# zhen6618/EPRecon

Measured on AMD Instinct MI355X. Metric: fragments_per_sec, higher is better.
Workload: dtype f32

## Files before the change

### eprecon_amd/_lib.py

```python
import ctypes
import os

import torch

_HERE = os.path.dirname(os.path.abspath(__file__))
LIB_PATH = os.environ.get("EPRECON_LIB_PATH") or os.path.join(_HERE, "libeprecon_hip.so")

_c = ctypes
_vp, _i, _i64, _f, _sz = _c.c_void_p, _c.c_int, _c.c_int64, _c.c_float, _c.c_size_t

SIGNATURES = {
    "eprecon_abi_version": (_i, []),
    "eprecon_build_arch": (_c.c_char_p, []),
    "eprecon_back_project_workspace_bytes": (_sz, [_i64, _i, _i, _i, _i, _i, _i]),
    "eprecon_back_project_async": (_i, [_vp, _i64, _vp, _i, _f, _vp, _i, _vp, _i, _i, _i, _i, _i, _i,
                                        _vp, _vp, _vp, _vp, _vp, _vp, _vp, _vp, _sz, _vp]),
    "eprecon_back_project": (_i, [_vp, _i64, _vp, _i, _f, _vp, _i, _vp, _i, _i, _i, _i, _i, _i, _i,
                                  _vp, _vp, _vp, _vp, _vp, _vp, _vp, _vp, _vp, _sz, _vp]),
    "eprecon_profile_gather_kernel": (_c.c_char_p, []),
    "eprecon_hash_capacity": (_c.c_uint32, [_i64]),
    "eprecon_hash_table_bytes": (_sz, [_c.c_uint32]),
    "eprecon_hash_build_async": (_i, [_vp, _i64, _i, _vp, _c.c_uint32, _vp]),
    "eprecon_hash_build_dn_async": (_i, [_vp, _i64, _vp, _i, _vp, _c.c_uint32, _vp]),
    "eprecon_hash_query_async": (_i, [_vp, _c.c_uint32, _vp, _i64, _i, _vp, _vp]),
    "eprecon_hash_status": (_i, [_vp, _vp]),
    "eprecon_unique_workspace_bytes": (_sz, [_i64]),
    "eprecon_unique_coords_async": (_i, [_vp, _i64, _i, _vp, _c.c_uint32, _vp, _vp, _vp, _vp, _sz, _vp]),
    "eprecon_unique_coords_dn_async": (_i, [_vp, _i64, _vp, _i, _vp, _c.c_uint32, _vp, _vp, _vp, _vp, _sz, _vp]),
    "eprecon_unique_hierarchy_dn_async": (_i, [_vp, _i64, _vp, _i, _vp, _vp, _vp, _vp, _vp, _vp, _sz, _vp]),
    "eprecon_point_quantize_dn_async": (_i, [_vp, _i64, _vp, _f, _vp, _vp, _vp]),
    "eprecon_spvcnn_points_dn_async": (_i, [_vp, _i64, _vp, _i, _i, _vp, _i, _f, _vp, _f, _vp, _vp, _vp, _vp, _vp, _vp]),
    "eprecon_gru_stage_capacity": (_i64, [_vp, _i64, _i]),
    "eprecon_gru_stage_workspace_bytes": (_sz, [_i64]),
    "eprecon_gru_stage_begin_async": (_i, [_vp, _vp]),
    "eprecon_gru_stage_commit_async": (_i, [_vp, _vp, _vp, _vp]),
    "eprecon_kernel_map_async": (_i, [_vp, _c.c_uint32, _vp, _i64, _i, _i, _vp, _vp]),
    "eprecon_kernel_map_self_async": (_i, [_vp, _c.c_uint32, _vp, _i64, _i, _vp, _vp]),
    "eprecon_transpose_map_async": (_i, [_vp, _i64, _vp, _i, _vp, _vp]),
    "eprecon_sparse_conv_async": (_i, [_vp, _i64, _i, _vp, _i, _i64, _vp, _i, _i, _vp, _vp, _i, _i, _i, _vp]),
    "eprecon_conv_bn_partial_bytes": (_sz, [_i64, _i]),
    "eprecon_sparse_conv_fused_async": (_i, [_vp, _i64, _i, _vp, _i, _i64, _vp, _i, _i, _vp, _vp, _i, _vp, _i, _i, _i,
                                             _vp, _vp]),
    "eprecon_conv_desc_async": (_i, [_vp, _vp]),
    "eprecon_exclusive_scan_async": (_i, [_vp, _i64, _vp, _vp, _vp, _vp]),
    "eprecon_conv_desc_partial_rows": (_i64, [_vp]),
    "eprecon_bn_acc_words": (_sz, [_i]),
    "eprecon_conv_desc_takes_bn_acc": (_i, [_vp]),
    "eprecon_batchnorm_acc_affine_async": (_i, [_vp, _i, _i, _i, _f, _vp, _vp, _vp]),
    "eprecon_affine_rows_acc_async": (_i, [_vp, _i64, _i, _i, _vp, _i, _i, _f, _i, _vp, _i, _vp]),
# ... 402 lines not shown
```

### eprecon_amd/back_project.py

```python
import ctypes

import torch
import torch.nn as nn

from . import _lib

MODE_MEAN, MODE_MEAN_DEPTH, MODE_VARIANCE = 0, 1, 2
LAYOUT_NCHW, LAYOUT_NHWC = 0, 1
def mark_dense(coords, dims, interval, batch=1):
    coords._eprecon_dense = (tuple(int(d) for d in dims), int(interval), int(batch))
    return coords


def _prep_feats(feats):
    v, b, c, h, w = feats.shape
    if feats.dtype != torch.float32:
        feats = feats.float()
    want = (b * h * w * c, h * w * c, 1, w * c, c)
    if all(sz == 1 or st == ws for sz, st, ws in zip(feats.shape, feats.stride(), want)):
        return feats, LAYOUT_NHWC
    return feats.contiguous(), LAYOUT_NCHW


class PendingBackProject:
# ... 150 lines not shown
    res = run(coords, origin, voxel_size, feats, KRcam, min_view_number, MODE_MEAN, min_valid_per_batch=0)
    if res is None:
        return torch.empty((0, feats.shape[2]), dtype=feats.dtype, device=feats.device)
    return res["feats"]


def forward_behind(module, coords, origin, voxel_size, feats, KRcam, min_view_number, behind):
    pend = run_async(coords, origin, voxel_size, feats, KRcam, min_view_number, MODE_MEAN, want_grid=module.return_projection,
                     hold_read=True, extra_words=behind.n_extra)
    nb = pend.n_valid_dev.numel() - behind.n_extra
    finish = behind(pend.coords_all, pend.n_valid_dev[0:1], pend.n_valid_dev[nb:])
    host = _lib.read_counts(pend.n_valid_dev)
    res = pend.result_from(host[:nb])
    if res is None:
        return None, None
    out_coords = res["coords"] if coords.dtype == torch.int32 else res["coords"].to(coords.dtype)
    return [res["feats"], out_coords, res.get("grid"), res.get("mask"), res["count"]], finish(res["n_valid"], host[nb:])


def view_variance(coords, origin, voxel_size, feats_fused, KRcam, min_view_number, min_valid=1000):
    if torch.is_grad_enabled() and feats_fused.requires_grad:
        from . import autograd as AG
        res = AG.back_project(coords, origin, voxel_size, feats_fused, KRcam, min_view_number, MODE_VARIANCE,
                              min_valid_per_batch=min_valid, want_mean=True)
    else:
        res = run(coords, origin, voxel_size, feats_fused, KRcam, min_view_number, MODE_VARIANCE,
                  min_valid_per_batch=min_valid, want_mean=True)
    if res is None:
        return None
    res["var"] = res.pop("feats")
    return res


def to_channels_last(feats):
    lib = _lib.load()
    v, b, c, h, w = feats.shape
    src = feats.float().contiguous()
    dst = torch.empty((v, b, h, w, c), dtype=torch.float32, device=feats.device)
    _lib.check(lib.eprecon_nchw_to_nhwc_async(_lib.ptr(src), _lib.ptr(dst), v * b, c, h * w,
                                               _lib.current_stream()), "eprecon_nchw_to_nhwc_async")
    return dst.permute(0, 1, 4, 2, 3)
```

### eprecon_amd/csrc/back_project.hip

```cpp
#include <stdlib.h>

#include "common.hpp"

namespace {
using namespace ep;


struct BpParams {
    const int32_t *coords;
    int n;
    const float *origin;
    int batch;
    float voxel_size;
    const float *feats_nhwc;
    const float *krcam;
    int V, C, H, W;
    int Cs;
    int min_view;
    float *out_feats;
    float *out_mean;
    int32_t *out_coords;
    float *count;
    float *out_grid;
    uint8_t *out_mask;
    int32_t *n_valid_dev;
    int32_t *block_offsets;
    int xcd_slabs;
};

struct Proj {
    float gx, gy, pz;
    bool vis;
};

__device__ __forceinline__ Proj project(const float *P, float X, float Y, float Z, float wm1,
                                        float hm1)
{
    const float px = __fmaf_rn(P[3], 1.0f, __fmaf_rn(P[2], Z, __fmaf_rn(P[1], Y, __fmul_rn(P[0], X))));
    const float py = __fmaf_rn(P[7], 1.0f, __fmaf_rn(P[6], Z, __fmaf_rn(P[5], Y, __fmul_rn(P[4], X))));
    const float pz = __fmaf_rn(P[11], 1.0f, __fmaf_rn(P[10], Z, __fmaf_rn(P[9], Y, __fmul_rn(P[8], X))));
    const float u = __fdiv_rn(px, pz);
    const float v = __fdiv_rn(py, pz);
    Proj r;
    r.gx = __fsub_rn(__fdiv_rn(__fmul_rn(2.0f, u), wm1), 1.0f);
    r.gy = __fsub_rn(__fdiv_rn(__fmul_rn(2.0f, v), hm1), 1.0f);
    r.pz = pz;
    r.vis = (fabsf(r.gx) <= 1.0f) && (fabsf(r.gy) <= 1.0f) && (pz > 0.0f);
    return r;
}

struct ProjFast {
    float u, v, pz;
    bool vis;
};

__device__ __forceinline__ ProjFast project_fast(const float *P, float X, float Y, float Z, float wm1, float hm1,
                                                 float kx, float ky)
{
    const float px = __fmaf_rn(P[3], 1.0f, __fmaf_rn(P[2], Z, __fmaf_rn(P[1], Y, __fmul_rn(P[0], X))));
// ... 117 lines not shown
        }
        if (lane == kWave - 1) sWave[wid] = x;
        __syncthreads();
        int woff = 0, tot = 0;
#pragma unroll
        for (int w = 0; w < 1024 / kWave; ++w) {
            const int c = sWave[w];
            woff += (w < wid) ? c : 0;
            tot += c;
        }
        if (i < nblk) block_sums[i] = carry + woff + x - v;
        carry += tot;
        __syncthreads();
    }
    if (tid == 0) n_valid_dev[0] = carry;
    if (batch == 1) {
        if (tid == 0) n_valid_dev[1] = carry;
    } else if (blk_batch) {
        for (int b = 0; b < batch; ++b) {
            int x = 0;
            for (int i = tid; i < nblk_count; i += 1024) x += blk_batch[(size_t)i * batch + b];
#pragma unroll
            for (int d = kWave / 2; d > 0; d >>= 1) x += __shfl_xor(x, d);
            __syncthreads();
            if (lane == 0) sWave[wid] = x;
            __syncthreads();
            if (tid == 0) {
                int t = 0;
                for (int w = 0; w < 1024 / kWave; ++w) t += sWave[w];
                n_valid_dev[1 + b] = t;
            }
        }
    }
}

struct Taps {
    int o00, o10, o01, o11;
    float w00, w10, w01, w11;
};

__device__ __forceinline__ Taps make_taps(float ix, float iy, int W, int H, int C)
{
    const float x0f = floorf(ix), y0f = floorf(iy);
    int x0 = (int)x0f, y0 = (int)y0f;
    float wx1 = ix - x0f, wx0 = (x0f + 1.0f) - ix;
    float wy1 = iy - y0f, wy0 = (y0f + 1.0f) - iy;
    int x1 = x0 + 1, y1 = y0 + 1;
    if (x1 >= W) { x1 = W - 1; wx1 = 0.0f; }
    if (y1 >= H) { y1 = H - 1; wy1 = 0.0f; }
    Taps t;
    t.o00 = (y0 * W + x0) * C;
    t.o10 = (y0 * W + x1) * C;
    t.o01 = (y1 * W + x0) * C;
    t.o11 = (y1 * W + x1) * C;
    t.w00 = wx0 * wy0;
    t.w10 = wx1 * wy0;
    t.w01 = wx0 * wy1;
    t.w11 = wx1 * wy1;
    return t;
}

template <int VEC>
struct Chan;
template <>
struct Chan<4> {
    float4 v;
// ... 32 lines not shown
};
template <>
struct Chan<1> {
    float v;
    __device__ __forceinline__ static Chan zero() { return Chan{0.f}; }
    __device__ __forceinline__ static Chan sample(const float *m, const Taps &t)
    {
        return Chan{fmaf(m[t.o11], t.w11, fmaf(m[t.o01], t.w01, fmaf(m[t.o10], t.w10, m[t.o00] * t.w00)))};
    }
    __device__ __forceinline__ void add(const Chan &o) { v += o.v; }
    __device__ __forceinline__ void add_sqdiff(const Chan &f, const Chan &mean)
    {
        const float d = f.v - mean.v;
        v = fmaf(d, d, v);
    }
    __device__ __forceinline__ Chan div(float d) const { return Chan{__fdiv_rn(v, d)}; }
    __device__ __forceinline__ void store(float *dst, bool) const { dst[0] = v; }
};

template <int VOX, int MODE, int VEC, int QT>
__global__ __launch_bounds__(256) void bp_gather_kernel(BpParams p)
{
    extern __shared__ __attribute__((aligned(16))) char smem[];
    constexpr int BLOCK = 256;
    float2 *sPix = reinterpret_cast<float2 *>(smem);
    float *sP = reinterpret_cast<float *>(sPix + VOX * p.V);
    const int nP = (p.V * p.batch * 12 + 3) & ~3;
    uint32_t *sVis = reinterpret_cast<uint32_t *>(sP + nP);
    float *sDen = reinterpret_cast<float *>(sVis + VOX);
    int *sBatch = reinterpret_cast<int *>(sDen + VOX);
    int *sSlot = sBatch + VOX;
    int *sOut = sSlot + VOX;
    int *sWave = sOut + VOX;

    const int tid = threadIdx.x;
    const int lb = p.xcd_slabs ? xcd_remap(blockIdx.x, gridDim.x) : (int)blockIdx.x;
    stage_matrices(sP, p.krcam, p.V * p.batch, tid, BLOCK);
    __syncthreads();

    const int e = lb * VOX + tid;
    const int i = e;
    const float wm1 = (float)(p.W - 1), hm1 = (float)(p.H - 1);
    bool valid = false;
    int4 c = make_int4(0, 0, 0, 0);
    float X = 0.f, Y = 0.f, Z = 0.f, zsum = 0.f;
    int cnt = 0;
    uint32_t vis = 0;
    if (tid < VOX && e < p.n) {
        c = reinterpret_cast<const int4 *>(p.coords)[i];
        if (c.x >= 0 && c.x < p.batch) {
            voxel_centre(c, p.origin, p.voxel_size, X, Y, Z);
            for (int v = 0; v < p.V; ++v) {
                const Proj pr = project(sP + (v * p.batch + c.x) * 12, X, Y, Z, wm1, hm1);
                const float ix = __fmul_rn(__fdiv_rn(__fadd_rn(pr.gx, 1.0f), 2.0f), wm1);
                const float iy = __fmul_rn(__fdiv_rn(__fadd_rn(pr.gy, 1.0f), 2.0f), hm1);
                sPix[tid * p.V + v] = make_float2(ix, iy);
                if (pr.vis) {
                    vis |= 1u << v;
                    cnt += 1;
                    zsum += pr.pz;
                }
            }
            valid = cnt >= p.min_view;
        }
    }
    int nloc;
    const int rank = block_exclusive_rank<BLOCK>(valid, sWave, nloc);
    if (nloc == 0) return;
    const int base = p.block_offsets[lb];
    const int n_valid = p.n_valid_dev[0];
    const int cout = (MODE == EPRECON_BP_MEAN_DEPTH) ? p.C + 1 : p.C;
    if (valid) {
        const int o = base + rank;
        sSlot[rank] = tid;
        sOut[tid] = o;
        sVis[tid] = vis;
        const float den = (float)(cnt > 0 ? cnt : 1);
        sDen[tid] = den;
        sBatch[tid] = c.x;
        reinterpret_cast<int4 *>(p.out_coords)[o] = c;
        if (MODE == EPRECON_BP_MEAN_DEPTH) p.out_feats[(size_t)o * cout + p.C] = __fdiv_rn(zsum, den);
        if (p.out_grid || p.out_mask) {
            for (int v = 0; v < p.V; ++v) {
                const Proj pr = project(sP + (v * p.batch + c.x) * 12, X, Y, Z, wm1, hm1);
                if (p.out_grid)
                    reinterpret_cast<float2 *>(p.out_grid)[(size_t)v * n_valid + o] = make_float2(pr.gx, pr.gy);
                if (p.out_mask) p.out_mask[(size_t)v * n_valid + o] = pr.vis ? 1 : 0;
            }
        }
    }
    __syncthreads();

    const int Q = QT > 0 ? QT : p.C / VEC;
    const size_t map_elems = (size_t)p.H * p.W * p.Cs;
    const bool aligned16 = (MODE != EPRECON_BP_MEAN_DEPTH);
    for (int w = tid; w < nloc * Q; w += BLOCK) {
        const int r = w / Q;
        const int q = w - r * Q;
        const int t = sSlot[r];
        const uint32_t vm = sVis[t];
        const float den = sDen[t];
        const int b = sBatch[t];
        const float *fb = p.feats_nhwc + (size_t)b * map_elems + q * VEC;
// ... 55 lines not shown
            a[u] = __builtin_amdgcn_raw_buffer_load_b128(rsrc, off[u], 0, 0);
            b[u] = __builtin_amdgcn_raw_buffer_load_b128(rsrc, off[u], s10, 0);
            c[u] = __builtin_amdgcn_raw_buffer_load_b128(rsrc, off[u], s01, 0);
            d[u] = __builtin_amdgcn_raw_buffer_load_b128(rsrc, off[u], s11, 0);
        }
#pragma unroll
        for (int u = 0; u < U; ++u) {
            const float wx1 = wxy[u].x, wy1 = wxy[u].y;
            const float wx0 = 1.0f - wx1, wy0 = 1.0f - wy1;
            const float w00 = wx0 * wy0, w10 = wx1 * wy0, w01 = wx0 * wy1, w11 = wx1 * wy1;
            float4 r;
#define EP_TAP(k) fmaf(__uint_as_float(d[u].k), w11, fmaf(__uint_as_float(c[u].k), w01, fmaf(__uint_as_float(b[u].k), w10, __uint_as_float(a[u].k) * w00)))
            r.x = EP_TAP(x); r.y = EP_TAP(y); r.z = EP_TAP(z); r.w = EP_TAP(w);
#undef EP_TAP
            if (on[u]) f(r);
        }
    }
}

template <int VOX, int MODE, int QT, int U>
__global__ __launch_bounds__(256) void bp_gather_mlp_kernel(BpParams p)
{
    extern __shared__ __attribute__((aligned(16))) char smem[];
    constexpr int BLOCK = 256;
    constexpr int VPT = BLOCK / VOX;
    float2 *sWxy = reinterpret_cast<float2 *>(smem);
    int *sOff = reinterpret_cast<int *>(sWxy + VOX * p.V);
    float *sP = reinterpret_cast<float *>(sOff + VOX * p.V);
    const int nP = (p.V * p.batch * 12 + 3) & ~3;
    uint32_t *sVis = reinterpret_cast<uint32_t *>(sP + nP);
    int *sSlot = reinterpret_cast<int *>(sVis + VOX);
    int *sOut = sSlot + VOX;
    int *sWave = sOut + VOX;

    const int tid = threadIdx.x;
    const int lb = p.xcd_slabs ? xcd_remap(blockIdx.x, gridDim.x) : (int)blockIdx.x;
    stage_matrices(sP, p.krcam, p.V * p.batch, tid, BLOCK);
    if (VPT > 1 && tid < VOX) sVis[tid] = 0;
    __syncthreads();

    const float wm1 = (float)(p.W - 1), hm1 = (float)(p.H - 1);
    const float kx = 2.0f / wm1, ky = 2.0f / hm1;
    const int map_elems = p.H * p.W * p.Cs;
    const int vx = tid % VOX;
    const int e = lb * VOX + vx;
    int4 c = make_int4(-1, 0, 0, 0);
    if (e < p.n) c = reinterpret_cast<const int4 *>(p.coords)[e];
    const bool in_batch = c.x >= 0 && c.x < p.batch;
    uint32_t vis = 0;
    if (in_batch) {
        float X, Y, Z;
        voxel_centre(c, p.origin, p.voxel_size, X, Y, Z);
        for (int v = tid / VOX; v < p.V; v += VPT) {
            const ProjFast q = project_fast(sP + (v * p.batch + c.x) * 12, X, Y, Z, wm1, hm1, kx, ky);
            if (!q.vis) continue;
            const float x0f = fminf(floorf(q.u), wm1 - 1.0f), y0f = fminf(floorf(q.v), hm1 - 1.0f);
            sWxy[vx * p.V + v] = make_float2(q.u - x0f, q.v - y0f);
            sOff[vx * p.V + v] = ((v * p.batch + c.x) * map_elems + ((int)y0f * p.W + (int)x0f) * p.Cs) * 4;
            vis |= 1u << v;
        }
        if (VPT > 1 && vis) atomicOr(&sVis[vx], vis);
    }
    if (VPT > 1) {
        __syncthreads();
        vis = sVis[vx];
    }
    const int cnt = __popc(vis);
    const bool valid = tid < VOX && in_batch && cnt >= p.min_view;
    int nloc;
    const int rank = block_exclusive_rank<BLOCK>(valid, sWave, nloc);
    if (nloc == 0) return;
    const int n_valid = p.n_valid_dev[0];
    const int cout = (MODE == EPRECON_BP_MEAN_DEPTH) ? p.C + 1 : p.C;
    if (valid) {
        const int o = p.block_offsets[lb] + rank;
        sSlot[rank] = tid;
        sOut[tid] = o;
        if (VPT == 1) sVis[tid] = vis;
        reinterpret_cast<int4 *>(p.out_coords)[o] = c;
        if (MODE == EPRECON_BP_MEAN_DEPTH || p.out_grid || p.out_mask) {
            float X, Y, Z, zsum = 0.0f;
            voxel_centre(c, p.origin, p.voxel_size, X, Y, Z);
            for (int v = 0; v < p.V; ++v) {
                const Proj pr = project(sP + (v * p.batch + c.x) * 12, X, Y, Z, wm1, hm1);
                if (pr.vis) zsum += pr.pz;
                if (p.out_grid)
                    reinterpret_cast<float2 *>(p.out_grid)[(size_t)v * n_valid + o] = make_float2(pr.gx, pr.gy);
                if (p.out_mask) p.out_mask[(size_t)v * n_valid + o] = pr.vis ? 1 : 0;
            }
            if (MODE == EPRECON_BP_MEAN_DEPTH)
                p.out_feats[(size_t)o * cout + p.C] = __fdiv_rn(zsum, (float)(cnt > 0 ? cnt : 1));
        }
    }
    __syncthreads();
    const __amdgpu_buffer_rsrc_t rsrc = __builtin_amdgcn_make_buffer_rsrc(
        const_cast<float *>(p.feats_nhwc), 0, p.V * p.batch * map_elems * 4, 0x00020000);
    const int Q = QT > 0 ? QT : p.C / 4;
    const int s10 = p.Cs * 4, s01 = p.W * p.Cs * 4, s11 = s01 + s10;
    for (int w = tid; w < nloc * Q; w += BLOCK) {
        const int r = w / Q, q = w - r * Q;
        const int t = sSlot[r];
        const uint32_t vm = sVis[t];
        const float den = (float)max(__popc(vm), 1);
        const int *offRow = sOff + t * p.V;
        const float2 *wxyRow = sWxy + t * p.V;
        float4 acc = make_float4(0.f, 0.f, 0.f, 0.f);
        visit_visible_samples<U>(rsrc, offRow, wxyRow, vm, q * 16, s10, s01, s11, [&](const float4 &f) {
            acc.x += f.x; acc.y += f.y; acc.z += f.z; acc.w += f.w;
// ... 34 lines not shown
    auto block_sum = [&](float x) -> float {
#pragma unroll
        for (int s = kWave / 2; s > 0; s >>= 1) x += __shfl_xor(x, s);
        __syncthreads();
        if (lane == 0) sRed[wid] = x;
        __syncthreads();
        float t = 0.f;
#pragma unroll
        for (int w = 0; w < 1024 / kWave; ++w) t += sRed[w];
        return t;
    };
    float s = 0.f, m = 0.f;
    for (int j = tid; j < len; j += 1024) {
        const float x = d[(size_t)j * cout];
        if (x > 0.f) { s += x; m += 1.f; }
    }
    const float tot = block_sum(s), cntp = block_sum(m);
    const float mu = tot / cntp;
    float ss = 0.f;
    for (int j = tid; j < len; j += 1024) {
        const float x = d[(size_t)j * cout];
        if (x > 0.f) ss = fmaf(x - mu, x - mu, ss);
    }
    const float sigma = sqrtf(block_sum(ss)) + 1e-5f;
    for (int j = tid; j < len; j += 1024) {
        const float x = d[(size_t)j * cout];
        d[(size_t)j * cout] = x > 0.f ? (x - mu) / sigma : 0.f;
    }
    (void)sBcast;
}

constexpr int kTrPix = 64;
__global__ __launch_bounds__(256) void nchw_to_nhwc_kernel(const float *__restrict__ in,
                                                           float *__restrict__ out, int C, int hw, int Cs,
                                                           int32_t *zero = nullptr, int zero_n = 0)
{
    extern __shared__ __attribute__((aligned(16))) char smem[];
    float *tile = reinterpret_cast<float *>(smem);
    if (blockIdx.x == 0 && blockIdx.y == 0 && (int)threadIdx.x < zero_n) zero[threadIdx.x] = 0;
    const int map = blockIdx.y;
    const int p0 = blockIdx.x * kTrPix;
    const int npix = min(kTrPix, hw - p0);
    const float *src = in + (size_t)map * C * hw;
    float *dst = out + (size_t)map * hw * Cs + (size_t)p0 * Cs;
    for (int e = threadIdx.x; e < C * kTrPix; e += 256) {
        const int c = e / kTrPix, px = e - c * kTrPix;
        if (px < npix) tile[c * (kTrPix + 1) + px] = src[(size_t)c * hw + p0 + px];
    }
    __syncthreads();
    for (int e = threadIdx.x; e < npix * Cs; e += 256) {
        const int px = e / Cs, c = e - px * Cs;
        dst[e] = c < C ? tile[c * (kTrPix + 1) + px] : 0.0f;
    }
}


struct ViewsParams {
    eprecon_views_desc d;
    int tile0[4];
    int tiles[3];
};
__global__ __launch_bounds__(256) void views_to_rows_kernel(ViewsParams p)
{
    extern __shared__ __attribute__((aligned(16))) char smem[];
    float *tile = reinterpret_cast<float *>(smem);
    const int b = blockIdx.x;
    const int l = b >= p.tile0[2] ? 2 : (b >= p.tile0[1] ? 1 : 0);
    const int r = b - p.tile0[l];
    const int v = r / p.tiles[l], t = r - v * p.tiles[l];
    const int C = p.d.channels[l], hw = p.d.hw[l];
    const int p0 = t * kTrPix;
    const int npix = min(kTrPix, hw - p0);
// ... 78 lines not shown
        const float iy = __fmul_rn(__fdiv_rn(__fadd_rn(pr.gy, 1.0f), 2.0f), hm1);
        const Taps t = make_taps(ix, iy, p.W, p.H, p.C);
        const size_t mo = ((size_t)v * p.batch + c.x) * map_elems + ch;
        float gv;
        if (p.mode == EPRECON_BP_VARIANCE) {
            const float f = Chan<1>::sample(p.feats_nhwc + mo, t).v;
            gv = 2.0f * (f - mean) * inv * g + gm;
        } else {
            gv = g * inv;
        }
        if (p.dfix) {
            unsigned long long *d = p.dfix + mo;
            float *m = p.dfeats + mo;
            if (t.w00 != 0.0f) fixed_add(d + t.o00, m + t.o00, t.w00 * gv);
            if (t.w10 != 0.0f) fixed_add(d + t.o10, m + t.o10, t.w10 * gv);
            if (t.w01 != 0.0f) fixed_add(d + t.o01, m + t.o01, t.w01 * gv);
            if (t.w11 != 0.0f) fixed_add(d + t.o11, m + t.o11, t.w11 * gv);
        } else {
            float *d = p.dfeats + mo;
            if (t.w00 != 0.0f) unsafeAtomicAdd(d + t.o00, t.w00 * gv);
            if (t.w10 != 0.0f) unsafeAtomicAdd(d + t.o10, t.w10 * gv);
            if (t.w01 != 0.0f) unsafeAtomicAdd(d + t.o01, t.w01 * gv);
            if (t.w11 != 0.0f) unsafeAtomicAdd(d + t.o11, t.w11 * gv);
        }
    }
}

struct ProfileState {
    bool on = false, recorded = false, one_shot = false;
    hipEvent_t start = nullptr, stop = nullptr;
    const char *kernel = "";
} g_prof;

size_t gather_lds_bytes(int vox, int V, int B)
{
    const size_t nP = ((size_t)V * B * 12 + 3) & ~(size_t)3;
    return (size_t)vox * V * sizeof(float2) + nP * sizeof(float) + (size_t)vox * 5 * 4 +
           (size_t)(256 / kWave) * 4 + 16;
}

template <int VOX, int MODE>
int launch_gather(const BpParams &p, int nblk, hipStream_t st)
{
    const size_t lds = gather_lds_bytes(VOX, p.V, p.batch);
    const dim3 grid(nblk), block(256);
#define EP_GATHER(VEC, QT) hipLaunchKernelGGL((bp_gather_kernel<VOX, MODE, VEC, QT>), grid, block, lds, st, p)
    if (p.C % 4 == 0) {
        switch (p.C / 4) {
            case 6: EP_GATHER(4, 6); break;
            case 8: EP_GATHER(4, 8); break;
            case 10: EP_GATHER(4, 10); break;
            case 20: EP_GATHER(4, 20); break;
            default: EP_GATHER(4, 0); break;
        }
    } else {
        EP_GATHER(1, 0);
    }
#undef EP_GATHER
    EP_LAUNCH_CHECK();
    return EPRECON_OK;
}

size_t gather_mlp_lds_bytes(int vox, int V, int B)
{
    const size_t nP = ((size_t)V * B * 12 + 3) & ~(size_t)3;
    return (size_t)vox * V * 12 + nP * sizeof(float) + (size_t)vox * 3 * 4 + (size_t)(256 / kWave) * 4 + 16;
}

bool gather_mlp_supported(const BpParams &p)
{
    return p.C % 4 == 0 && p.Cs % 4 == 0 && p.V <= 32 &&
           (size_t)p.V * p.batch * p.H * p.W * p.Cs * 4 < 0x7fff0000ull &&
           gather_mlp_lds_bytes(256, p.V, p.batch) <= 64 * 1024;
}

template <int VOX, int MODE, int U>
int launch_gather_mlp_u(const BpParams &p, int nblk, hipStream_t st)
{
    const size_t lds = gather_mlp_lds_bytes(VOX, p.V, p.batch);
    const dim3 grid(nblk), block(256);
#define EP_GATHER(QT) hipLaunchKernelGGL((bp_gather_mlp_kernel<VOX, MODE, QT, U>), grid, block, lds, st, p)
    switch (p.C / 4) {
        case 6: EP_GATHER(6); break;
        case 8: EP_GATHER(8); break;
        case 10: EP_GATHER(10); break;
        case 20: EP_GATHER(20); break;
        default: EP_GATHER(0); break;
    }
#undef EP_GATHER
    EP_LAUNCH_CHECK();
    return EPRECON_OK;
}

template <int VOX, int MODE>
int launch_gather_mlp(const BpParams &p, int nblk, hipStream_t st)
{
    return launch_gather_mlp_u<VOX, MODE, 1>(p, nblk, st);
}

// ... 63 lines not shown
    if (lds > 64 * 1024) return EPRECON_ERR_UNSUPPORTED;
    const dim3 grid((unsigned)ep::ceil_div(hw, kTrPix), (unsigned)maps);
    hipLaunchKernelGGL(nchw_to_nhwc_kernel, grid, dim3(256), lds, (hipStream_t)stream, in, out,
                       channels, hw, channels);
    EP_LAUNCH_CHECK();
    return EPRECON_OK;
}

int eprecon_views_to_rows_async(const eprecon_views_desc *desc, void *stream)
{
    if (!desc || desc->levels < 1 || desc->levels > 3 || desc->n_views < 1 || desc->n_views > 16) return EPRECON_ERR_ARG;
    ViewsParams p = {};
    p.d = *desc;
    int cmax = 0, at = 0;
    for (int l = 0; l < 3; ++l) {
        p.tile0[l] = at;
        if (l >= desc->levels) { p.tiles[l] = 1; continue; }
        if (desc->channels[l] <= 0 || desc->hw[l] <= 0 || !desc->dst[l]) return EPRECON_ERR_ARG;
        for (int v = 0; v < desc->n_views; ++v)
            if (!desc->src[l][v]) return EPRECON_ERR_ARG;
        p.tiles[l] = ep::ceil_div(desc->hw[l], kTrPix);
        at += p.tiles[l] * desc->n_views;
        cmax = desc->channels[l] > cmax ? desc->channels[l] : cmax;
    }
    p.tile0[3] = at;
    for (int l = desc->levels; l < 3; ++l) p.tile0[l] = at;
    const size_t lds = (size_t)cmax * (kTrPix + 1) * sizeof(float);
    if (lds > 64 * 1024) return EPRECON_ERR_UNSUPPORTED;
    hipLaunchKernelGGL(views_to_rows_kernel, dim3((unsigned)at), dim3(256), lds, (hipStream_t)stream, p);
    EP_LAUNCH_CHECK();
    return EPRECON_OK;
}

int eprecon_back_project_async(const int32_t *coords, int64_t n, const float *origin, int batch,
                               float voxel_size, const float *feats, int feats_layout,
                               const float *krcam, int n_views, int channels, int height,
                               int width, int min_view, int mode, float *out_feats,
                               float *out_mean, int32_t *out_coords, float *count,
                               float *out_grid, uint8_t *out_mask, int32_t *n_valid_dev,
                               void *workspace, size_t workspace_bytes, void *stream)
{
    hipStream_t st = (hipStream_t)stream;
    if (n < 0 || n > 0x7fffffff / 64 || batch <= 0 || n_views <= 0 || n_views > 32 || channels <= 0 ||
        height <= 1 || width <= 1 || mode < 0 || mode > 2)
        return EPRECON_ERR_ARG;
    if (!origin || !feats || !krcam || !n_valid_dev || !workspace) return EPRECON_ERR_ARG;
    if (n > 0 && (!coords || !out_feats || !out_coords || !count)) return EPRECON_ERR_ARG;
    if ((size_t)n_views * batch * 12 * sizeof(float) > 32 * 1024) return EPRECON_ERR_UNSUPPORTED;
    if (workspace_bytes < eprecon_back_project_workspace_bytes(n, batch, n_views, channels, height,
                                                               width, feats_layout))
        return EPRECON_ERR_WORKSPACE;
    if ((size_t)n_views * batch * channels * height * width > 0x7fffffffull) return EPRECON_ERR_UNSUPPORTED;

    const bool clear_in_relayout = n > 0 && feats_layout == EPRECON_LAYOUT_NCHW && batch < 256;
    if (!clear_in_relayout) EP_HIP_CHECK(hipMemsetAsync(n_valid_dev, 0, sizeof(int32_t) * (size_t)(1 + batch), st));
    if (n == 0) return EPRECON_OK;

    char *ws = reinterpret_cast<char *>(workspace);
    int32_t *block_sums = reinterpret_cast<int32_t *>(ws);
    ws += ep::align_up((size_t)ep::ceil_div(n, 16) * sizeof(int32_t), 256);
    int32_t *blk_batch = reinterpret_cast<int32_t *>(ws);
    ws += ep::align_up((size_t)ep::ceil_div(n, 256) * batch * sizeof(int32_t), 256);
    const float *nhwc = feats;
    int pix_stride = channels;
    if (feats_layout == EPRECON_LAYOUT_NCHW) {
        float *tmp = reinterpret_cast<float *>(ws);
        const size_t lds_t = (size_t)channels * (kTrPix + 1) * sizeof(float);
        if (lds_t > 64 * 1024) return EPRECON_ERR_UNSUPPORTED;
        hipLaunchKernelGGL(nchw_to_nhwc_kernel, dim3((unsigned)ep::ceil_div(height * width, kTrPix), (unsigned)(n_views * batch)),
                           dim3(256), lds_t, st, feats, tmp, channels, height * width, pix_stride, n_valid_dev, 1 + batch);
        EP_LAUNCH_CHECK();
        nhwc = tmp;
        ws += ep::align_up((size_t)n_views * batch * pix_stride * height * width * sizeof(float), 256);
    } else if (feats_layout != EPRECON_LAYOUT_NHWC) {
        return EPRECON_ERR_ARG;
    }

    BpParams p;
    p.coords = coords; p.n = (int)n; p.origin = origin; p.batch = batch; p.voxel_size = voxel_size;
    p.feats_nhwc = nhwc; p.krcam = krcam; p.V = n_views; p.C = channels; p.Cs = pix_stride; p.H = height; p.W = width;
    p.min_view = min_view; p.out_feats = out_feats; p.out_mean = out_mean; p.out_coords = out_coords;
    p.count = count; p.out_grid = out_grid; p.out_mask = out_mask; p.n_valid_dev = n_valid_dev;
    p.block_offsets = block_sums;
    {
        const char *e = getenv("EPRECON_BP_XCD_SLABS");
        p.xcd_slabs = (e && e[0] == '0') ? 0 : 1;
    }

    const int vox = n >= 512 * 1024 ? 256 : (n >= 48 * 1024 ? 64 : 16);
    const int ntile = (int)ep::ceil_div(n, vox);
    const int nblk_count = (int)ep::ceil_div(n, 256);
    const size_t lds_count = ((size_t)n_views * batch * 12 + batch + 256 / ep::kWave) * 4 + 16;
    int32_t *bb = batch > 1 ? blk_batch : nullptr;
    if (vox == 256)
        hipLaunchKernelGGL((bp_count_kernel<256>), dim3(nblk_count), dim3(256), lds_count, st, p, block_sums, bb);
    else if (vox == 64)
        hipLaunchKernelGGL((bp_count_kernel<64>), dim3(nblk_count), dim3(256), lds_count, st, p, block_sums, bb);
    else
        hipLaunchKernelGGL((bp_count_kernel<16>), dim3(nblk_count), dim3(256), lds_count, st, p, block_sums, bb);
    EP_LAUNCH_CHECK();
    hipLaunchKernelGGL(bp_scan_kernel, dim3(1), dim3(1024), 0, st, block_sums, ntile, n_valid_dev,
                       (const int32_t *)bb, nblk_count, batch);
    EP_LAUNCH_CHECK();

    const bool prof = g_prof.on && g_prof.start;
    if (prof) EP_HIP_CHECK(hipEventRecord(g_prof.start, st));
    int rc;
#define EP_MODE_DISPATCH(VOX)                                                                        \
    rc = mode == EPRECON_BP_MEAN ? launch_gather<VOX, EPRECON_BP_MEAN>(p, ntile, st)                   \
       : mode == EPRECON_BP_MEAN_DEPTH ? launch_gather<VOX, EPRECON_BP_MEAN_DEPTH>(p, ntile, st)       \
                                       : launch_gather<VOX, EPRECON_BP_VARIANCE>(p, ntile, st)
#define EP_MODE_DISPATCH_MLP(VOX)                                                                    \
    rc = mode == EPRECON_BP_MEAN ? launch_gather_mlp<VOX, EPRECON_BP_MEAN>(p, ntile, st)               \
       : mode == EPRECON_BP_MEAN_DEPTH ? launch_gather_mlp<VOX, EPRECON_BP_MEAN_DEPTH>(p, ntile, st)   \
                                       : launch_gather_mlp<VOX, EPRECON_BP_VARIANCE>(p, ntile, st)
    if (gather_mlp_supported(p)) {
        if (vox == 256) { EP_MODE_DISPATCH_MLP(256); }
        else if (vox == 64) { EP_MODE_DISPATCH_MLP(64); }
        else { EP_MODE_DISPATCH_MLP(16); }
    }
    else if (vox == 256) { EP_MODE_DISPATCH(256); }
    else if (vox == 64) { EP_MODE_DISPATCH(64); }
    else { EP_MODE_DISPATCH(16); }
#undef EP_MODE_DISPATCH
#undef EP_MODE_DISPATCH_MLP
    if (rc != EPRECON_OK) return rc;
    if (prof) {
        EP_HIP_CHECK(hipEventRecord(g_prof.stop, st));
        g_prof.recorded = true;
        g_prof.kernel = gather_mlp_supported(p) ? "bp_gather_mlp_kernel" : "bp_gather_kernel";
        if (g_prof.one_shot) g_prof.on = false;
    }
    if (mode == EPRECON_BP_MEAN_DEPTH) {
        hipLaunchKernelGGL(bp_depth_norm_kernel, dim3(batch), dim3(1024), 0, st, out_feats,
                           channels + 1, n_valid_dev);
        EP_LAUNCH_CHECK();
// ... 83 lines not shown
```

### eprecon_amd/csrc/kernel_map.hip

```cpp
#include <stdlib.h>

#include <atomic>

#include "hashgrid.hpp"

namespace {
using namespace ep;

constexpr int kScanBlock = 256;
constexpr int kScanItems = 8;
constexpr int kScanTile = kScanBlock * kScanItems;

__global__ __launch_bounds__(kScanBlock) void scan_tile_sums(const int32_t *in, int n, int32_t *sums, const int32_t *n_dev)
{
    __shared__ int sWave[kScanBlock / kWave];
    if (n_dev) n = min(n, *n_dev);
    const int base = blockIdx.x * kScanTile;
    int s = 0;
    for (int k = 0; k < kScanItems; ++k) {
        const int i = base + k * kScanBlock + threadIdx.x;
        if (i < n) s += in[i];
    }
#pragma unroll
    for (int d = kWave / 2; d > 0; d >>= 1) s += __shfl_xor(s, d);
// ... 754 lines not shown
{
    return kernel_map_self_impl(table, capacity, coords, n, stride, nbr, true, stream);
}
}

extern "C" {

int eprecon_kernel_map_self_async(const void *table, uint32_t capacity, const int32_t *coords, int64_t n, int stride, int32_t *nbr,
                                  void *stream)
{
    return kernel_map_self_impl(table, capacity, coords, n, stride, nbr, false, stream);
}


int eprecon_transpose_map_async(const int32_t *fine_coords, int64_t n, const int32_t *parent,
                                int fine_stride, int32_t *up_map, void *stream)
{
    if (n < 0 || fine_stride < 1 || (n > 0 && (!fine_coords || !parent || !up_map))) return EPRECON_ERR_ARG;
    if (n == 0) return EPRECON_OK;
    hipLaunchKernelGGL(transpose_map_kernel, dim3((unsigned)ceil_div(n, 256)), dim3(256), 0,
                       (hipStream_t)stream, reinterpret_cast<const int4 *>(fine_coords), (int)n, parent,
                       fine_stride, up_map);
    EP_LAUNCH_CHECK();
    return EPRECON_OK;
}

int eprecon_grid_rank_async(const int32_t *coords, int64_t n, int stride, int grid_x, int grid_y, int grid_z, int32_t *rank,
                            void *stream)
{
    if (n < 0 || stride < 1 || grid_x <= 0 || grid_y <= 0 || grid_z <= 0 || !rank || (n > 0 && !coords) ||
        (int64_t)grid_x * grid_y * grid_z > 0x7ffffff0 || n > 0x7fffffff)
        return EPRECON_ERR_ARG;
    const size_t cells = (size_t)grid_x * grid_y * grid_z;
    EP_HIP_CHECK(hipMemsetAsync(rank, 0xff, cells * sizeof(int32_t), (hipStream_t)stream));
    EP_HIP_CHECK(hipMemsetAsync(rank + cells, 0, sizeof(int32_t), (hipStream_t)stream));
    if (n == 0) return EPRECON_OK;
    hipLaunchKernelGGL(grid_rank_kernel, dim3((unsigned)ceil_div(n, 256)), dim3(256), 0, (hipStream_t)stream,
                       reinterpret_cast<const int4 *>(coords), (int)n, stride, grid_x, grid_y, grid_z, rank, rank + cells);
    EP_LAUNCH_CHECK();
    return EPRECON_OK;
}

int eprecon_pixel_map_async(int maps, int height, int width, int ksize, int32_t *nbr, void *stream)
{
    if (maps <= 0 || height <= 0 || width <= 0 || ksize < 1 || ksize > 7 || !(ksize & 1) || !nbr ||
        (int64_t)maps * height * width > 0x7fffffff)
        return EPRECON_ERR_ARG;
    const int n = maps * height * width;
    hipLaunchKernelGGL(pixel_map_kernel, dim3((unsigned)ceil_div(n, 256), ksize * ksize), dim3(256), 0,
                       (hipStream_t)stream, maps, height, width, ksize, nbr);
    EP_LAUNCH_CHECK();
    return EPRECON_OK;
}

}
```

### eprecon_amd/fragment_step.py

```python
import os

import torch

from . import _lib
from . import back_project as BP
from . import grid_ops as GO
from . import synthetic as S
from .config import CH_IMG, CH_INIT_DOWN, N_VIEWS
from .occupancy_initialization import Occupancy_Initialization

LEVELS = [("bp24", 2, 4, 2), ("bp48", 1, 2, 0), ("bp96", 0, 1, 0)]


class Cfg2Step:
    def __init__(self, seed=0, device=None, height=480, width=640, n_vox=(96, 96, 96)):
        self.device = device or torch.device("cuda")
        self.seed = seed
        self.window = S.make_window(seed=seed, width=width, height=height, n_vox=n_vox)
        self.shapes = S.pyramid_shapes(height, width)
        dev = self.device
        t = lambda a: torch.from_numpy(a).to(dev)
        self.origin = t(self.window["vol_origin_partial"][None].copy())
        self.voxel_size = self.window["voxel_size"]
        self.krcam = [t(self.window["proj_matrices"][:, l][:, None].copy()) for l in range(3)]
# ... 16 lines not shown
    @torch.no_grad()
    def run(self):
        issued = self._issue()
        if not self.defer_reads:
            return self._finish(issued)
        prev, self._inflight = self._inflight, issued
        return self._finish(prev) if prev is not None else {}

    def flush(self):
        if self._inflight is not None:
            prev, self._inflight = self._inflight, None
            return self._finish(prev)
        return self.last

    def _finish(self, issued):
        out, pending, select = issued
        if select is not None:
            out["stage0_coords"], _ = select.result()
        for name in pending:
            out[name] = pending[name].result()
        self.last = out
        return out

    def _issue(self):
        out = {}
        pending = {}
        main = torch.cuda.current_stream(self.device)
        side = self._bp_stream if self.bp_side_stream else main

        def queue_levels():
            if side is not main:
                side.wait_stream(main)
            with torch.cuda.stream(side):
                for name, lvl, interval, mv in LEVELS:
                    if self.profile_dominant and name == "bp96":
                        _lib.load().eprecon_profile_enable(2)
                    pending[name] = BP.run_async(self.coords[interval], self.origin, self.voxel_size, self.feats[lvl],
                                                 self.krcam[lvl], mv)

        if not self.levels_inside:
            queue_levels()
        init = self.init_net(self.coords[2], self.origin, self.voxel_size, self.features_init,
                             self.krcam[1], self.shape_init, 1, 2, between=queue_levels if self.levels_inside else None)
        out["init"] = init
        select = None
        if init is not None:
            select = GO.init_select_async(init[0], init[1], 1, dim=self.shape_init[0] // 2, cell=4)
        if side is not main:
            main.wait_stream(side)
        return out, pending, select

    def dominant_kernel_ms(self, lib):
        return float(lib.eprecon_profile_gather_ms())

    def dominant_kernel_bytes(self):
        c, h, w = self.shapes[0]
        n = self.coords[1].shape[0]
        nv = self.last["bp96"]["n_valid"] if self.last.get("bp96") else n
        return 16 * n + 4 * N_VIEWS * c * h * w + nv * (4 * c + 16)

    def dominant_kernel_l1_bandwidth(self, launch_ms):
        if not launch_ms:
            return None
        c = self.shapes[0][0]
        n = self.coords[1].shape[0]
        nv = self.last["bp96"]["n_valid"] if self.last.get("bp96") else n
        req = float(nv) * N_VIEWS * 4 * 4 * c
        peak = 64.0 * 256 * 2.4e9 / 1e12
        ach = req / (launch_ms * 1e-3) / 1e12
        return {"requested_bytes": req, "requested_note": "upper bound: every valid voxel visible in all views (4 taps x 4 C bytes per view)",
# ... 282 lines not shown
```

### eprecon_amd/neucon_network.py

```python
import sys

import numpy as np
import torch
import torch.nn as nn

from . import _lib
from . import grid_ops as GO
from . import sparse as SP
from .back_project import Back_Project
from .backbone import stack_views
from .criterion import HungarianMatcher, SetCriterion, compute_loss, compute_loss_init
from .config import (CH_IMG, CH_INIT_DOWN, CH_VOXEL, EXCEED_NUM, INIT_MIN_VIEW, INIT_OCC_THRESHOLD, INIT_STAGE,
                     N_VIEWS, NUM_CLASSES, NUM_QUERIES, PANOPTIC_CH, PANOPTIC_SHAPE, STAGE_MIN_OCC)
from .generate_grids import dense_coords
from .gru_fusion import GRUFusion
from .mask3dformer import MultiScaleMaskedTransformerDecoder, panoptic_post
from .modules import Linear4xTrans, Panoptic_Feat_Fusion, SPVCNN, linear4x_pair
from .occupancy_initialization import Occupancy_Initialization
from .tensor import PointTensor
from .torchsparse_utils import SpvcnnPrefetch, aligned_camera_coords

_FUSED_SPARSIFY = True
_PREFETCH = __import__("os").environ.get("EPRECON_PREFETCH", "1") == "1"

# ... 133 lines not shown
        recording = torch.is_grad_enabled()
        zero = features[0][0].sum() * 0.0 if recording and features[0][0].requires_grad else torch.zeros((), device=dev)
        if self.distributed_exchange and cfg.FUSION.FUSION_ON:
            for b in range(bs):
                self.gru_fusion.exchange_boundaries(inputs, b)

        scale = self.n_scales - INIT_STAGE
        init_output, coord_init_selected, shape_init = self._init_stage(features, inputs, bs, dev, select=not only_train_init)
        if init_output is None:
            loss_dict["occupancy_initialization_loss"] = zero
            _warn("no valid points in initialization")
            outputs["init_overlap_count"] = init_overlap_count
            return outputs, loss_dict
        occ_init, coord_init, count_init = init_output
        if only_train_init:
            tsdf_init_target, occ_init_target = self.get_target_init(coord_init, inputs, scale)
            hit = occ_init.detach().sigmoid().reshape(-1) > INIT_OCC_THRESHOLD
            losses = []
            for b in range(bs):
                rows = coord_init[:, 0] == b
                pred, tgt = hit[rows], tsdf_init_target[rows] > 0
                init_overlap_count = init_overlap_count + (pred & tgt).sum() / (pred | tgt).sum()
                losses.append(compute_loss_init(occ_init[rows], tsdf_init_target[rows], occ_init_target[rows]))
            outputs["init_overlap_count"] = init_overlap_count
            loss_dict["occupancy_initialization_loss"] = sum(losses) / len(losses)
            return outputs, loss_dict
        self._record(stage="init", occ_init=occ_init, coord_init=coord_init, selected=coord_init_selected)

        pre_feat = pre_coords = None
        panoptic_voxel_feats, panoptic_coords = [], []
        occ_target = occupancy = None
        prefetch = _PREFETCH and dev.type == "cuda" and not recording and _FUSED_SPARSIFY
        ahead = pruned = None
        for i in range(cfg.N_LAYER):
            interval = 2 ** (self.n_scales - i)
            scale = self.n_scales - i
            ready, ahead = ahead, None
            if i == 0:
                up_coords = coord_init_selected.contiguous()
                min_view_number = 2
                up_feat = None
            else:
                if ready is not None and ready[0] is not None and ready[0].shape[0] == 8 * pre_coords.shape[0]:
                    up_feat, up_coords = GO.upsample(pre_feat, pre_coords, interval, up_coords=ready[0])
                else:
                    ready = None
                    up_feat, up_coords = self.upsample(pre_feat, pre_coords, interval)
                min_view_number = 0
            feats = stack_views([f[scale] for f in features_backbone2d_occ_pano])
            KRcam = inputs["proj_matrices"][:, :, scale].permute(1, 0, 2, 3).contiguous()
            if i == 0 and prefetch and up_coords.dtype == torch.int32:
                from . import back_project as BP
                project_output, ready = BP.forward_behind(self.back_projection[0], up_coords, inputs["vol_origin_partial"],
                                                          cfg.VOXEL_SIZE, feats, KRcam, min_view_number,
                                                          self._spvcnn_behind(0, inputs, children=False))
            else:
                project_output = self.back_projection[i](up_coords, inputs["vol_origin_partial"], cfg.VOXEL_SIZE,
                                                         feats, KRcam, min_view_number)
            if project_output is None:
                loss_dict[f"tsdf_occ_loss_{i}"] = zero
                _warn(f"no valid points in back_projection: scale {i}")
                return outputs, loss_dict
            volume, up_coords, _, _, count = project_output
            if i != 0:
                if min_view_number <= 0:
                    feat = torch.cat([volume, up_feat], dim=1)
                else:
                    keep = count >= min_view_number
                    feat = torch.cat([volume, up_feat if bool(keep.all()) else up_feat[keep]], dim=1)
            else:
                feat = volume

            if ready is not None and ready[1].shape[0] == up_coords.shape[0]:
                r_coords = ready[1]
            else:
                r_coords = aligned_camera_coords(up_coords, inputs["vol_origin_partial"], cfg.VOXEL_SIZE,
                                                 inputs["world_to_aligned_camera"])
            sp_in = feat
            feat = self.sp_convs[i](PointTensor(feat.contiguous(), r_coords))
            feat_all = torch.cat([feat, volume], dim=-1)
            self._record(stage=f"spvcnn{i}", coords=up_coords, feat_in=sp_in, r_coords=r_coords, feat_out=feat,
                         volume=volume)
# ... 204 lines not shown
```

### include/eprecon_hip.h

```cpp
#ifndef EPRECON_HIP_H
#define EPRECON_HIP_H

#include <stddef.h>
#include <stdint.h>

#ifdef __cplusplus
extern "C" {
#endif

#define EPRECON_OK 0
#define EPRECON_EMPTY 1
#define EPRECON_ERR_ARG (-1)
#define EPRECON_ERR_WORKSPACE (-2)
#define EPRECON_ERR_UNSUPPORTED (-3)
#define EPRECON_ERR_HIP_BASE (-1000)

#define EPRECON_ABI_VERSION 1
int eprecon_abi_version(void);
const char *eprecon_build_arch(void);

#define EPRECON_BP_MEAN 0
#define EPRECON_BP_MEAN_DEPTH 1
#define EPRECON_BP_VARIANCE 2

#define EPRECON_LAYOUT_NCHW 0
#define EPRECON_LAYOUT_NHWC 1

size_t eprecon_back_project_workspace_bytes(int64_t n, int batch, int n_views, int channels,
                                            int height, int width, int feats_layout);

int eprecon_back_project_async(const int32_t *coords, int64_t n, const float *origin, int batch,
                               float voxel_size, const float *feats, int feats_layout,
                               const float *krcam, int n_views, int channels, int height,
                               int width, int min_view, int mode, float *out_feats,
                               float *out_mean, int32_t *out_coords, float *count,
                               float *out_grid, uint8_t *out_mask, int32_t *n_valid_dev,
                               void *workspace, size_t workspace_bytes, void *stream);

int eprecon_back_project(const int32_t *coords, int64_t n, const float *origin, int batch,
                         float voxel_size, const float *feats, int feats_layout,
                         const float *krcam, int n_views, int channels, int height, int width,
                         int min_view, int mode, int min_valid_per_batch, float *out_feats,
                         float *out_mean, int32_t *out_coords, float *count, float *out_grid,
                         uint8_t *out_mask, int32_t *n_valid_dev, int32_t *n_valid_host,
                         void *workspace, size_t workspace_bytes, void *stream);

int eprecon_profile_enable(int on);
float eprecon_profile_gather_ms(void);
const char *eprecon_profile_gather_kernel(void);

int eprecon_profile_conv_arm(int kvol, int cin, int cout, int64_t min_rows);
float eprecon_profile_conv_ms(int64_t *rows_out, const char **kernel_out);
int64_t eprecon_profile_conv_pairs(void);
int64_t eprecon_profile_conv_executed_pairs(void);
const char *eprecon_profile_last_conv_kernel(void);
int eprecon_profile_mark_async(int id, void *stream);

int eprecon_nchw_to_nhwc_async(const float *in, float *out, int maps, int channels, int hw,
                               void *stream);
typedef struct eprecon_views_desc {
    const float *src[3][16];
    float *dst[3];
    int32_t channels[3]; int32_t hw[3];
    int32_t levels; int32_t n_views;
} eprecon_views_desc;
int eprecon_views_to_rows_async(const eprecon_views_desc *desc, void *stream);

uint32_t eprecon_hash_capacity(int64_t n);
size_t eprecon_hash_table_bytes(uint32_t capacity);
int eprecon_hash_build_async(const int32_t *coords, int64_t n, int quantum, void *table,
// ... 418 lines not shown
```

Before: 746.7.

## Fuse tile prefix into gather kernels and batch multi-level feature relayout

For single-batch back projection without grid or mask output, each gather block now sums the per-tile counts ahead of it, so the separate single-block scan kernel launch is skipped. The last tile writes the valid total. Feature maps for all levels are converted to channels-last in one batched relayout call rather than one call per level. Grid-rank initialisation uses a multi-region fill instead of two memsets. The cost is redundant prefix reads per block, which grow with tile count and are capped at a maximum, plus extra LDS.

```diff
diff --git a/eprecon_amd/_lib.py b/eprecon_amd/_lib.py
--- a/eprecon_amd/_lib.py
+++ b/eprecon_amd/_lib.py
@@ -15,6 +15,7 @@
     "eprecon_back_project_workspace_bytes": (_sz, [_i64, _i, _i, _i, _i, _i, _i]),
     "eprecon_back_project_async": (_i, [_vp, _i64, _vp, _i, _f, _vp, _i, _vp, _i, _i, _i, _i, _i, _i,
                                         _vp, _vp, _vp, _vp, _vp, _vp, _vp, _vp, _sz, _vp]),
+    "eprecon_back_project_prefix_max_tiles": (_i, []),
     "eprecon_back_project": (_i, [_vp, _i64, _vp, _i, _f, _vp, _i, _vp, _i, _i, _i, _i, _i, _i, _i,
                                   _vp, _vp, _vp, _vp, _vp, _vp, _vp, _vp, _vp, _sz, _vp]),
     "eprecon_profile_gather_kernel": (_c.c_char_p, []),
diff --git a/eprecon_amd/back_project.py b/eprecon_amd/back_project.py
--- a/eprecon_amd/back_project.py
+++ b/eprecon_amd/back_project.py
@@ -206,6 +206,27 @@
     return res
 
 
+def relayout_levels(feats_list):
+    feats_list = list(feats_list)
+    maps = feats_list[0].shape[0] * feats_list[0].shape[1]
+    if (not 1 <= len(feats_list) <= 3 or maps > 16 or feats_list[0].device.type != "cuda"
+            or any(f.shape[0] * f.shape[1] != maps for f in feats_list)):
+        return [to_channels_last(f) for f in feats_list]
+    src = [f.float().contiguous() for f in feats_list]
+    d = _lib.ViewsDesc()
+    d.levels, d.n_views = len(src), maps
+    out = []
+    for l, f in enumerate(src):
+        v, b, c, h, w = f.shape
+        dst = torch.empty((v, b, h, w, c), dtype=torch.float32, device=f.device)
+        d.channels[l], d.hw[l], d.dst[l] = c, h * w, dst.data_ptr()
+        for m in range(maps):
+            d.src[l][m] = f.data_ptr() + m * c * h * w * 4
+        out.append(dst.permute(0, 1, 4, 2, 3))
+    _lib.check(_lib.load().eprecon_views_to_rows_async(ctypes.byref(d), _lib.current_stream()), "eprecon_views_to_rows_async")
+    return out
+
+
 def to_channels_last(feats):
     lib = _lib.load()
     v, b, c, h, w = feats.shape
diff --git a/eprecon_amd/csrc/back_project.hip b/eprecon_amd/csrc/back_project.hip
--- a/eprecon_amd/csrc/back_project.hip
+++ b/eprecon_amd/csrc/back_project.hip
@@ -25,6 +25,7 @@
     uint8_t *out_mask;
     int32_t *n_valid_dev;
     int32_t *block_offsets;
+    int tile_prefix;
     int xcd_slabs;
 };
 
@@ -208,6 +209,43 @@
             }
         }
     }
+}
+
+__device__ __forceinline__ int tile_prefix_partial(const BpParams &p, int lb, int tid)
+{
+    if (!p.tile_prefix) return 0;
+    const int32_t *t = p.block_offsets;
+    int s = 0;
+    for (int i = tid; i < lb; i += 4 * 256) {
+        const int a = t[i];
+        const int b = i + 256 < lb ? t[i + 256] : 0;
+        const int c = i + 512 < lb ? t[i + 512] : 0;
+        const int d = i + 768 < lb ? t[i + 768] : 0;
+        s += (a + b) + (c + d);
+    }
+    return s;
+}
+
+__device__ __forceinline__ void tile_prefix_stage(const BpParams &p, int part, int *red, int tid)
+{
+    if (!p.tile_prefix) return;
+#pragma unroll
+    for (int d = kWave / 2; d > 0; d >>= 1) part += __shfl_xor(part, d);
+    if ((tid & (kWave - 1)) == 0) red[tid / kWave] = part;
+}
+
+__device__ __forceinline__ int tile_base(const BpParams &p, const int *red, int lb, int nloc, int ntile, int tid)
+{
+    if (!p.tile_prefix) return nloc ? p.block_offsets[lb] : 0;
+    int base = 0;
+#pragma unroll
+    for (int w = 0; w < 256 / kWave; ++w) base += red[w];
+    if (lb == ntile - 1 && tid == 0) {
+        const int total = base + nloc;
+        p.n_valid_dev[0] = total;
+        p.n_valid_dev[1] = total;
+    }
+    return base;
 }
 
 struct Taps {
@@ -306,9 +344,11 @@
     int *sSlot = sBatch + VOX;
     int *sOut = sSlot + VOX;
     int *sWave = sOut + VOX;
+    int *sRed = sWave + BLOCK / kWave;
 
     const int tid = threadIdx.x;
     const int lb = p.xcd_slabs ? xcd_remap(blockIdx.x, gridDim.x) : (int)blockIdx.x;
+    const int part = tile_prefix_partial(p, lb, tid);
     stage_matrices(sP, p.krcam, p.V * p.batch, tid, BLOCK);
     __syncthreads();
 
@@ -339,10 +379,11 @@
         }
     }
     int nloc;
+    tile_prefix_stage(p, part, sRed, tid);
     const int rank = block_exclusive_rank<BLOCK>(valid, sWave, nloc);
+    const int base = tile_base(p, sRed, lb, nloc, (int)gridDim.x, tid);
     if (nloc == 0) return;
-    const int base = p.block_offsets[lb];
-    const int n_valid = p.n_valid_dev[0];
+    const int n_valid = (p.out_grid || p.out_mask) ? p.n_valid_dev[0] : 0;
     const int cout = (MODE == EPRECON_BP_MEAN_DEPTH) ? p.C + 1 : p.C;
     if (valid) {
         const int o = base + rank;
@@ -464,9 +505,11 @@
     int *sSlot = reinterpret_cast<int *>(sVis + VOX);
     int *sOut = sSlot + VOX;
     int *sWave = sOut + VOX;
+    int *sRed = sWave + BLOCK / kWave;
 
     const int tid = threadIdx.x;
     const int lb = p.xcd_slabs ? xcd_remap(blockIdx.x, gridDim.x) : (int)blockIdx.x;
+    const int part = tile_prefix_partial(p, lb, tid);
     stage_matrices(sP, p.krcam, p.V * p.batch, tid, BLOCK);
     if (VPT > 1 && tid < VOX) sVis[tid] = 0;
     __syncthreads();
@@ -500,12 +543,14 @@
     const int cnt = __popc(vis);
     const bool valid = tid < VOX && in_batch && cnt >= p.min_view;
     int nloc;
+    tile_prefix_stage(p, part, sRed, tid);
     const int rank = block_exclusive_rank<BLOCK>(valid, sWave, nloc);
+    const int base = tile_base(p, sRed, lb, nloc, (int)gridDim.x, tid);
     if (nloc == 0) return;
-    const int n_valid = p.n_valid_dev[0];
+    const int n_valid = (p.out_grid || p.out_mask) ? p.n_valid_dev[0] : 0;
     const int cout = (MODE == EPRECON_BP_MEAN_DEPTH) ? p.C + 1 : p.C;
     if (valid) {
-        const int o = p.block_offsets[lb] + rank;
+        const int o = base + rank;
         sSlot[rank] = tid;
         sOut[tid] = o;
         if (VPT == 1) sVis[tid] = vis;
@@ -606,12 +651,10 @@
 
 constexpr int kTrPix = 64;
 __global__ __launch_bounds__(256) void nchw_to_nhwc_kernel(const float *__restrict__ in,
-                                                           float *__restrict__ out, int C, int hw, int Cs,
-                                                           int32_t *zero = nullptr, int zero_n = 0)
+                                                           float *__restrict__ out, int C, int hw, int Cs)
 {
     extern __shared__ __attribute__((aligned(16))) char smem[];
     float *tile = reinterpret_cast<float *>(smem);
-    if (blockIdx.x == 0 && blockIdx.y == 0 && (int)threadIdx.x < zero_n) zero[threadIdx.x] = 0;
     const int map = blockIdx.y;
     const int p0 = blockIdx.x * kTrPix;
     const int npix = min(kTrPix, hw - p0);
@@ -756,11 +799,16 @@
     const char *kernel = "";
 } g_prof;
 
+#ifndef EP_BP_PREFIX_MAX_TILES
+#define EP_BP_PREFIX_MAX_TILES 4096
+#endif
+constexpr int kPrefixMaxTiles = EP_BP_PREFIX_MAX_TILES;
+
 size_t gather_lds_bytes(int vox, int V, int B)
 {
     const size_t nP = ((size_t)V * B * 12 + 3) & ~(size_t)3;
     return (size_t)vox * V * sizeof(float2) + nP * sizeof(float) + (size_t)vox * 5 * 4 +
-           (size_t)(256 / kWave) * 4 + 16;
+           (size_t)(256 / kWave) * 4 * 2 + 16;
 }
 
 template <int VOX, int MODE>
@@ -788,7 +836,7 @@
 size_t gather_mlp_lds_bytes(int vox, int V, int B)
 {
     const size_t nP = ((size_t)V * B * 12 + 3) & ~(size_t)3;
-    return (size_t)vox * V * 12 + nP * sizeof(float) + (size_t)vox * 3 * 4 + (size_t)(256 / kWave) * 4 + 16;
+    return (size_t)vox * V * 12 + nP * sizeof(float) + (size_t)vox * 3 * 4 + (size_t)(256 / kWave) * 4 * 2 + 16;
 }
 
 bool gather_mlp_supported(const BpParams &p)
@@ -918,6 +966,8 @@
     return EPRECON_OK;
 }
 
+int eprecon_back_project_prefix_max_tiles(void) { return kPrefixMaxTiles; }
+
 int eprecon_back_project_async(const int32_t *coords, int64_t n, const float *origin, int batch,
                                float voxel_size, const float *feats, int feats_layout,
                                const float *krcam, int n_views, int channels, int height,
@@ -938,9 +988,10 @@
         return EPRECON_ERR_WORKSPACE;
     if ((size_t)n_views * batch * channels * height * width > 0x7fffffffull) return EPRECON_ERR_UNSUPPORTED;
 
-    const bool clear_in_relayout = n > 0 && feats_layout == EPRECON_LAYOUT_NCHW && batch < 256;
-    if (!clear_in_relayout) EP_HIP_CHECK(hipMemsetAsync(n_valid_dev, 0, sizeof(int32_t) * (size_t)(1 + batch), st));
-    if (n == 0) return EPRECON_OK;
+    if (n == 0) {
+        EP_HIP_CHECK(hipMemsetAsync(n_valid_dev, 0, sizeof(int32_t) * (size_t)(1 + batch), st));
+        return EPRECON_OK;
+    }
 
     char *ws = reinterpret_cast<char *>(workspace);
     int32_t *block_sums = reinterpret_cast<int32_t *>(ws);
@@ -954,7 +1005,7 @@
         const size_t lds_t = (size_t)channels * (kTrPix + 1) * sizeof(float);
         if (lds_t > 64 * 1024) return EPRECON_ERR_UNSUPPORTED;
         hipLaunchKernelGGL(nchw_to_nhwc_kernel, dim3((unsigned)ep::ceil_div(height * width, kTrPix), (unsigned)(n_views * batch)),
-                           dim3(256), lds_t, st, feats, tmp, channels, height * width, pix_stride, n_valid_dev, 1 + batch);
+                           dim3(256), lds_t, st, feats, tmp, channels, height * width, pix_stride);
         EP_LAUNCH_CHECK();
         nhwc = tmp;
         ws += ep::align_up((size_t)n_views * batch * pix_stride * height * width * sizeof(float), 256);
@@ -976,6 +1027,7 @@
     const int vox = n >= 512 * 1024 ? 256 : (n >= 48 * 1024 ? 64 : 16);
     const int ntile = (int)ep::ceil_div(n, vox);
     const int nblk_count = (int)ep::ceil_div(n, 256);
+    p.tile_prefix = (batch == 1 && !out_grid && !out_mask && ntile <= kPrefixMaxTiles) ? 1 : 0;
     const size_t lds_count = ((size_t)n_views * batch * 12 + batch + 256 / ep::kWave) * 4 + 16;
     int32_t *bb = batch > 1 ? blk_batch : nullptr;
     if (vox == 256)
@@ -985,9 +1037,11 @@
     else
         hipLaunchKernelGGL((bp_count_kernel<16>), dim3(nblk_count), dim3(256), lds_count, st, p, block_sums, bb);
     EP_LAUNCH_CHECK();
-    hipLaunchKernelGGL(bp_scan_kernel, dim3(1), dim3(1024), 0, st, block_sums, ntile, n_valid_dev,
-                       (const int32_t *)bb, nblk_count, batch);
-    EP_LAUNCH_CHECK();
+    if (!p.tile_prefix) {
+        hipLaunchKernelGGL(bp_scan_kernel, dim3(1), dim3(1024), 0, st, block_sums, ntile, n_valid_dev,
+                           (const int32_t *)bb, nblk_count, batch);
+        EP_LAUNCH_CHECK();
+    }
 
     const bool prof = g_prof.on && g_prof.start;
     if (prof) EP_HIP_CHECK(hipEventRecord(g_prof.start, st));
diff --git a/eprecon_amd/csrc/kernel_map.hip b/eprecon_amd/csrc/kernel_map.hip
--- a/eprecon_amd/csrc/kernel_map.hip
+++ b/eprecon_amd/csrc/kernel_map.hip
@@ -810,8 +810,9 @@
         (int64_t)grid_x * grid_y * grid_z > 0x7ffffff0 || n > 0x7fffffff)
         return EPRECON_ERR_ARG;
     const size_t cells = (size_t)grid_x * grid_y * grid_z;
-    EP_HIP_CHECK(hipMemsetAsync(rank, 0xff, cells * sizeof(int32_t), (hipStream_t)stream));
-    EP_HIP_CHECK(hipMemsetAsync(rank + cells, 0, sizeof(int32_t), (hipStream_t)stream));
+    const ep::FillRegion reg[2] = {{rank, cells * sizeof(int32_t), 0xffffffffu}, {rank + cells, sizeof(int32_t), 0u}};
+    const int rc = ep::multi_fill(reg, 2, (hipStream_t)stream);
+    if (rc != EPRECON_OK) return rc;
     if (n == 0) return EPRECON_OK;
     hipLaunchKernelGGL(grid_rank_kernel, dim3((unsigned)ceil_div(n, 256)), dim3(256), 0, (hipStream_t)stream,
                        reinterpret_cast<const int4 *>(coords), (int)n, stride, grid_x, grid_y, grid_z, rank, rank + cells);
diff --git a/eprecon_amd/fragment_step.py b/eprecon_amd/fragment_step.py
--- a/eprecon_amd/fragment_step.py
+++ b/eprecon_amd/fragment_step.py
@@ -72,10 +72,12 @@
             if side is not main:
                 side.wait_stream(main)
             with torch.cuda.stream(side):
+                feats = dict(zip((lvl for _, lvl, _, _ in LEVELS),
+                                 BP.relayout_levels([self.feats[lvl] for _, lvl, _, _ in LEVELS])))
                 for name, lvl, interval, mv in LEVELS:
                     if self.profile_dominant and name == "bp96":
                         _lib.load().eprecon_profile_enable(2)
-                    pending[name] = BP.run_async(self.coords[interval], self.origin, self.voxel_size, self.feats[lvl],
+                    pending[name] = BP.run_async(self.coords[interval], self.origin, self.voxel_size, feats[lvl],
                                                  self.krcam[lvl], mv)
 
         if not self.levels_inside:
diff --git a/eprecon_amd/neucon_network.py b/eprecon_amd/neucon_network.py
--- a/eprecon_amd/neucon_network.py
+++ b/eprecon_amd/neucon_network.py
@@ -189,6 +189,11 @@
         occ_target = occupancy = None
         prefetch = _PREFETCH and dev.type == "cuda" and not recording and _FUSED_SPARSIFY
         ahead = pruned = None
+        level_feats = None
+        if dev.type == "cuda" and not recording:
+            from . import back_project as BP
+            level_feats = BP.relayout_levels([stack_views([f[self.n_scales - i] for f in features_backbone2d_occ_pano])
+                                              for i in range(cfg.N_LAYER)])
         for i in range(cfg.N_LAYER):
             interval = 2 ** (self.n_scales - i)
             scale = self.n_scales - i
@@ -204,7 +209,10 @@
                     ready = None
                     up_feat, up_coords = self.upsample(pre_feat, pre_coords, interval)
                 min_view_number = 0
-            feats = stack_views([f[scale] for f in features_backbone2d_occ_pano])
+            if level_feats is not None:
+                feats = level_feats[i]
+            else:
+                feats = stack_views([f[scale] for f in features_backbone2d_occ_pano])
             KRcam = inputs["proj_matrices"][:, :, scale].permute(1, 0, 2, 3).contiguous()
             if i == 0 and prefetch and up_coords.dtype == torch.int32:
                 from . import back_project as BP
diff --git a/include/eprecon_hip.h b/include/eprecon_hip.h
--- a/include/eprecon_hip.h
+++ b/include/eprecon_hip.h
@@ -36,6 +36,7 @@
                                float *out_mean, int32_t *out_coords, float *count,
                                float *out_grid, uint8_t *out_mask, int32_t *n_valid_dev,
                                void *workspace, size_t workspace_bytes, void *stream);
+int eprecon_back_project_prefix_max_tiles(void);
 
 int eprecon_back_project(const int32_t *coords, int64_t n, const float *origin, int batch,
                          float voxel_size, const float *feats, int feats_layout,
```

Measured after the change: 756.8, median of 6. Within noise of the previous version (+1.4%).
